# duanyiqun/DiffusionDepth

Measured on AMD Instinct MI355X. Metric: depth-maps/sec (20-step DDIM, KITTI 352x1216 f16r, B=4 maps per GPU per step; depth RMSE vs the reference's CPU path <= 1e-3 on this workload AND at KITTI's depth range 0-80 m: see cpu_baseline.rmse_gate), higher is better.
Workload: dtype f16 (f16 MFMA operands, fp32 accumulation; refined mode: f16-pair weights in conv1 / conv4 / conv3(cond), block-scaled int16 hand-over of y3 and conv3(cond)); 1 GPU; kitti 352x1216 image -> latent 16x176x608, cond 256x176x608, Res head denoiser (mmbev_res50 config), T=20, encoder+loop+decoder, inputs resident in HBM; global_batch=4, parallelism=dp1 (independent images, no collective), ranks_seen=1, streams=2, graph=True, variant=res

## Files before the change

diffusiondepth_amd/csrc/dd_api.cpp:

```cpp
#include "dd_api_internal.h"
#include <cstdlib>

namespace ddapi {
thread_local std::string g_create_error;
}


extern "C" {

const char* dd_version(void) { return "ddepth 0.1 gfx950 (hip, mfma bf16/f16/f32 implicit-GEMM conv3x3+GN+ReLU, hipGraph DDIM loop)"; }

const char* dd_last_error(dd_handle_t h) { return h ? h->err.c_str() : g_create_error.c_str(); }

int dd_create(dd_handle_t* out, int device, int variant) {
  if (!out) { g_create_error = "dd_create: out is NULL"; return DD_ERR_INVALID_ARG; }
  *out = nullptr;
  if (variant != DD_VARIANT_RES && variant != DD_VARIANT_SWIN) { g_create_error = "dd_create: unknown variant"; return DD_ERR_INVALID_ARG; }
  int n = 0;
  hipError_t e = hipGetDeviceCount(&n);
  if (e != hipSuccess || n <= 0) {
    g_create_error = std::string("dd_create: no HIP device available (") + (e != hipSuccess ? hipGetErrorString(e) : "count = 0") +
                     "); this library has no CPU fallback";
    return DD_ERR_HIP;
  }
// ... 82 lines not shown
    h->swin_w5 = (int)value;
  }
  else if (k == "hoist_cond") {
    if (value < -1 || value > 1) return h->fail(DD_ERR_INVALID_ARG, "dd_set_option: hoist_cond must be -1 (automatic), 0 or 1");
    h->hoist_cond = (int)value;
  }
  else if (k == "bf16_storage") {
    if (h->bf16_pure != (value != 0)) {
      DD_HIP(hipDeviceSynchronize());
      h->plans.clear(); h->last_once_plan = nullptr;
      h->cond_bufs.clear(); h->fpn_cond.reset(); h->fpn_cond_key[3] = -1; h->fpn_out.reset(); h->fpn_work.reset();
    }
    h->bf16_pure = value != 0;
  }
  else if (k == "naive_wgrad") h->naive_wgrad = value != 0;
  else if (k == "lane_probe") h->lane_probe = value != 0;
  else if (k == "x3_grad_fp32") h->x3_grad_fp32 = value != 0;
  else if (k == "grad_autoscale") h->grad_autoscale = value != 0;
  else if (k == "keep_trajectory") h->keep_traj = value != 0;
  else if (k == "use_trajectory") h->use_traj = value;
  else if (k == "adjoint_tiled") h->adjoint_tiled = value != 0;
  else if (k == "streams") h->n_streams = value < 1 ? 1 : (int)value;
  else if (k == "keep_activations_mb") h->keep_act_mb = value < 0 ? 0 : value;
  else if (k == "big_tiles") {
    if (value < -1 || value > 1) return h->fail(DD_ERR_INVALID_ARG, "dd_set_option: big_tiles must be -1 (automatic), 0 or 1");
    if (h->big_tiles != (int)value) { DD_HIP(hipDeviceSynchronize()); h->plans.clear(); h->last_once_plan = nullptr; }
    h->big_tiles = (int)value;
  }
  else if (k == "thin_slots") {
    if (value < 1 || value > 4096) return h->fail(DD_ERR_INVALID_ARG, "dd_set_option: thin_slots must be in [1, 4096]");
    if (h->thin_slots != (int)value) { DD_HIP(hipDeviceSynchronize()); h->plans.clear(); h->last_once_plan = nullptr; }
    h->thin_slots = (int)value;
  }
  else if (k == "one_buffer") {
    if (value < 0 || value > 2) return h->fail(DD_ERR_INVALID_ARG, "dd_set_option: one_buffer must be 0, 1 or 2");
    if (h->one_buffer != (int)value) { DD_HIP(hipDeviceSynchronize()); h->plans.clear(); h->last_once_plan = nullptr; }
    h->one_buffer = (int)value;
  }
  else if (k == "cond_direct") {
    if (value < 0 || value > 1) return h->fail(DD_ERR_INVALID_ARG, "dd_set_option: cond_direct must be 0 or 1");
    h->cond_direct = (int)value;
  }
  else if (k == "cond_split") {
    if (value < 0 || value > 1) return h->fail(DD_ERR_INVALID_ARG, "dd_set_option: cond_split must be 0 or 1");
    h->cond_split = (int)value;
  }
  else if (k == "thin_stream") {
    if (value < 0 || value > 1) return h->fail(DD_ERR_INVALID_ARG, "dd_set_option: thin_stream must be 0 or 1");
    if (h->thin_stream != (int)value) {
      DD_HIP(hipDeviceSynchronize());
      h->plans.clear(); h->last_once_plan = nullptr;
    }
    h->thin_stream = (int)value;
  }
  else if (k == "f16r_wide" || k == "f16r_p4" || k == "f16r_c1") {
    if (value < 0 || value > 1) return h->fail(DD_ERR_INVALID_ARG, "dd_set_option: " + k + " must be 0 or 1");
    int& opt = k == "f16r_wide" ? h->f16r_wide : k == "f16r_c1" ? h->f16r_c1 : h->f16r_p4;
    if (opt != (int)value) { DD_HIP(hipDeviceSynchronize()); h->plans.clear(); h->last_once_plan = nullptr; }
    opt = (int)value;
  }
  else if (k == "phase_prof_buffer") h->prof_buf = reinterpret_cast<unsigned long long*>((uintptr_t)value);
  else if (k == "phase_prof_layer") h->prof_layer = (int)value;
  else if (k == "layer_timing") {
    drain_layer_events(h);
    h->layer_timing = value != 0;
    for (int i = 0; i < dd_handle_s::N_LAYER_SLOTS; ++i) { h->layer_ms[i] = 0; h->layer_cnt[i] = 0; }
  } else return h->fail(DD_ERR_INVALID_ARG, "dd_set_option: unknown key '" + k + "'");
  return DD_OK;
}

int dd_get_counter(dd_handle_t h, const char* key, int64_t* value) {
  if (!h || !key || !value) return DD_ERR_INVALID_ARG;
  const std::string k(key);
  if (k == "graph_launches") *value = h->n_graph_launches;
  else if (k == "graph_default") *value = h->graph_off_by_env ? 0 : 1;
  else if (k == "eager_loops") *value = h->n_eager_loops;
  else if (k == "graph_capture_failures") *value = h->n_capture_failures;
  else if (k == "plans") *value = (int64_t)h->plans.size();
  else if (k == "neck_launches") *value = h->n_neck_launches;
  else if (k == "trajectory_ticket") *value = h->traj_serial;
  else if (k == "lane_calls") *value = h->n_lane_calls;
  else if (k == "lane_probe_retries") *value = h->n_lane_probe_retries;
  else if (k == "lane_overlap") *value = h->lane_overlap_seen;
  else if (k == "cond_split_ok") *value = (h->fpn_committed && h->fpn_split_ok ? 1 : 0) | (h->neck_committed && h->neck_split_ok ? 2 : 0);
  else if (k == "resident_slots") *value = h->resident_slots;
  else if (k == "trajectory_reuses") *value = h->n_traj_reuse;
  else if (k == "thin_stream_launches") *value = h->thin_stream_launches;
  else if (k.compare(0, 13, "kid_launches:") == 0) {
    int id = 0;
    const size_t n = k.size() - 13;
    bool ok = n >= 1 && n <= 3 && !(n > 1 && k[13] == '0');
    for (size_t i = 13; ok && i < k.size(); ++i) { ok = k[i] >= '0' && k[i] <= '9'; id = id * 10 + (k[i] - '0'); }
    if (!ok || !kid_listed(id)) return h->fail(DD_ERR_INVALID_ARG, "dd_get_counter: '" + k + "' does not name a kernel id (dd_kernel_ids.h)");
    *value = h->kid_launches[id];
  }
  else return h->fail(DD_ERR_INVALID_ARG, "dd_get_counter: unknown key '" + k + "'");
  return DD_OK;
}

int dd_get_layer_ms(dd_handle_t h, int layer, double* total_ms, int64_t* launches) {
  if (!h || layer < 1 || layer > dd_handle_s::N_LAYER_SLOTS || !total_ms || !launches) return DD_ERR_INVALID_ARG;
  drain_layer_events(h);
  *total_ms = h->layer_ms[layer - 1];
  *launches = h->layer_cnt[layer - 1];
  return DD_OK;
}

int dd_last_loop_ms(dd_handle_t h, float* ms) {
  if (!h || !ms) return DD_ERR_INVALID_ARG;
  *ms = 0.f;
  if (!h->ev_valid) return DD_OK;
  DD_HIP(hipEventSynchronize(h->ev1));
  DD_HIP(hipEventElapsedTime(ms, h->ev0, h->ev1));
  return DD_OK;
}

static int condition_impl(dd_handle_t h, const float* const* feats, const int* feat_h, const int* feat_w, int n_levels, int B,
                          float* cond_out, int precision, void* stream, bool with_neck);

int dd_condition(dd_handle_t h, const float* const* feats, const int* feat_h, const int* feat_w, int n_levels, int B,
                 float* cond_out, int precision, void* stream) {
  return condition_impl(h, feats, feat_h, feat_w, n_levels, B, cond_out, precision, stream, false);
}

int dd_neck_condition(dd_handle_t h, const float* const* feats, const int* feat_h, const int* feat_w, int n_levels, int B,
                      float* cond_out, int precision, void* stream) {
  if (!h) return DD_ERR_INVALID_ARG;
  if (!h->neck_committed) return h->fail(DD_ERR_STATE, "hahineck.* weights not committed (dd_set_weight for the lateral / projection / fusion convolutions, "
                                                       "dd_commit_weights; DD_VARIANT_SWIN)");
  return condition_impl(h, feats, feat_h, feat_w, n_levels, B, cond_out, precision, stream, true);
}

static int condition_impl(dd_handle_t h, const float* const* feats, const int* feat_h, const int* feat_w, int n_levels, int B,
                          float* cond_out, int precision, void* stream, bool with_neck) {
  if (!h) return DD_ERR_INVALID_ARG;
  if (!h->fpn_committed) return h->fail(DD_ERR_STATE, "conv_lateral.* / conv_up.* weights not committed (dd_set_weight, dd_commit_weights)");
  if (with_neck && h->variant != DD_VARIANT_SWIN)
    return h->fail(DD_ERR_UNSUPPORTED, "dd_neck_condition: the HAHI neck kernels are built for the Swin-L (192/384/768/1536) and MPViT-small (128/216/288/288) pyramids of DD_VARIANT_SWIN");
  if (n_levels != FPN_LEVELS || !feats || !feat_h || !feat_w) return h->fail(DD_ERR_INVALID_ARG, "dd_condition: expects 4 pyramid levels");
  if (precision < DD_PREC_FP32 || precision > DD_PREC_LAST) return h->fail(DD_ERR_INVALID_ARG, "dd_condition: precision must be fp32, bf16, f16, f16x3 or f16r");
// ... 522 lines not shown
```

diffusiondepth_amd/csrc/dd_api_internal.h:

```cpp
#pragma once
#include "../../include/ddepth.h"
#include "dd_kernels.h"
#include "dd_kernel_ids.h"

#include <cmath>
#include <cstdio>
#include <cstring>
#include <list>
#include <map>
#include <memory>
#include <set>
#include <string>
#include <tuple>
#include <vector>

using namespace dd;

namespace ddapi {

extern thread_local std::string g_create_error;

struct DevBuf {
  void* p = nullptr;
  size_t bytes = 0;
// ... 41 lines not shown
enum { PYR_DEFAULT = 0, PYR_MPVIT = 1 };
inline int pyramid_of(int variant, int pyr) { return pyr == PYR_MPVIT ? PYRAMID_MPVIT : variant == DD_VARIANT_SWIN ? PYRAMID_SWIN : PYRAMID_RES; }
inline const int* fpn_cin(int variant, int pyr) {
  return pyr == PYR_MPVIT ? FPN_CIN_MPVIT : (variant == DD_VARIANT_SWIN ? FPN_CIN_SWIN : FPN_CIN_RES);
}
inline const int* fpn_cin_pad(int variant, int pyr) { return pyr == PYR_MPVIT ? FPN_CIN_MPVIT_PAD : fpn_cin(variant, pyr); }

struct ConvLayer {
  int cin = 0, cout = 0;
  DevBuf wpack2[NUM_WIMG];
  DevBuf bias;
  DevBuf w_oihw;
  DevBuf wpackT[NUM_EK];
  DevBuf wT_oihw;
  DevBuf gamma, beta;
};

struct PlanKey {
  int B, h, w, ch, cw, T, prec, hoist;
  int keep = 0;
  int lane = 0;
  int lanes = 1;
  bool operator<(const PlanKey& o) const {
    return std::tie(B, h, w, ch, cw, T, prec, hoist, keep, lane, lanes) < std::tie(o.B, o.h, o.w, o.ch, o.cw, o.T, o.prec, o.hoist, o.keep, o.lane, o.lanes);
  }
};

struct Plan {
  PlanKey key{};
  int ek = EK_F32;
  DevBuf x[2];
  std::shared_ptr<DevBuf> cond;
  const void* cond_alias = nullptr;
  const void* graph_cond = nullptr;
  void* cond_ptr() const { return cond_alias ? const_cast<void*>(cond_alias) : (cond ? cond->p : nullptr); }
  DevBuf y1, y2, y3, y4;
  DevBuf a1, f, a3, eps;
  DevBuf sa, sf;
  DevBuf bX, bA1, bF, bA3;
  DevBuf bSa, bSf;
  DevBuf xstash;
  int64_t traj_ticket = 0;
  int64_t traj_weights = -1;
  bool traj_consumed = false;
  DevBuf gA, gY;
  DevBuf dgb;
  DevBuf bcorr;
  DevBuf ttab, tt_scratch;
  int64_t ttab_weights = -1;
  DevBuf ccond;
  DevBuf ccond_raw;
  DevBuf ccond_scale;
  DevBuf y3_scale;
  bool wide = false, c1 = false, p4 = false;
  DevBuf stats;
  DevBuf c1c2;
  DevBuf tsteps;
  std::vector<long long> tsteps_host;
  size_t stats_bytes = 0;
  hipGraphExec_t exec = nullptr;
  bool capture_failed = false;
  uint64_t last_use = 0;
  ~Plan() { if (exec) (void)hipGraphExecDestroy(exec); }
  int slots = 1;
  size_t kept_bytes = 0;
  void* slot(const DevBuf& b, int step) const { return static_cast<char*>(b.p) + (slots > 1 ? (size_t)step * (b.bytes / slots) : 0); }
  double* stat_ptr(int step, int layer) const {
    return stats.as<double>() + ((size_t)(step * 4 + layer) * key.B) * STAT_SLOTS * STAT_STRIDE;
  }
};

struct FpnWork {
  int B = 0, ek = -1, pyr = 0, hs[FPN_LEVELS] = {0}, ws[FPN_LEVELS] = {0};
  DevBuf fin[FPN_LEVELS];
  DevBuf lat[FPN_LEVELS];
  DevBuf up[FPN_LEVELS - 1];
  DevBuf pooled[FPN_LEVELS - 1];
  bool neck = false;
  DevBuf nk_cat[FPN_LEVELS];
  DevBuf nk_out[FPN_LEVELS];
};


struct NeckConv { int layer; std::string name; int cout, cin, ks, level, kind, C, Ck; };
constexpr int NECK_C_MPVIT[4] = {128, 216, 288, 288};
inline int neck_c(int pyr, int level) { return pyr == PYR_MPVIT ? NECK_C_MPVIT[level] : (192 << level); }
inline int neck_ck(int pyr, int level) { return pyr == PYR_MPVIT ? FPN_CIN_MPVIT_PAD[level] : (192 << level); }
inline std::vector<NeckConv> neck_convs(int pyr) {
  std::vector<NeckConv> v;
  const int P = pyramid_of(DD_VARIANT_SWIN, pyr);
  for (int i = 0; i < 4; ++i) {
    const int C = neck_c(pyr, i), Ck = neck_ck(pyr, i);
    const std::string si = std::to_string(i), sj = std::to_string(i - 1);
    v.push_back({kid_neck(P, NECK_LATERAL, i), "hahineck.lateral_convs." + si, C, C, 1, i, NECK_LATERAL, C, Ck});
    v.push_back({kid_neck(P, NECK_PROJ, i), i == 0 ? std::string("hahineck.conv_proj.0") : "hahineck.trans_proj." + sj, 512, C, 1, i, NECK_PROJ, C, Ck});
    v.push_back({kid_neck(P, NECK_FUSION, i), i == 0 ? std::string("hahineck.conv_fusion.0") : "hahineck.trans_fusion." + sj, C, C + 512, 3, i, NECK_FUSION, C, Ck});
  }
  return v;
}

}
using namespace ddapi;


struct dd_handle_s {
  static constexpr int MAX_LANES = 4;
  int device = 0;
  int variant = DD_VARIANT_RES;
  std::string err;
  std::map<std::string, std::vector<float>> host_w;
  std::map<std::string, std::unique_ptr<DevBuf>> dev_w;
  std::set<std::string> dev_newer;
  DevBuf stage;
  bool committed = false;
  bool codec_committed = false;
  ConvLayer L[4];
  ConvLayer LA, LB;
  DevBuf emb;
  DevBuf etab;
  DevBuf w5_oihw, w5pack[NUM_WIMG], pairp, kside;
  int64_t w5_weights = -1;
  int swin_w5 = 1;
  DevBuf zero_bias;
  int hoist_cond = -1;
  bool bf16_pure = false;
  DevBuf codec_buf;
  CodecWeights codec{};
  DevBuf codec_tmp;
  std::vector<float> acp;
  DevBuf d_acp;
  int n_train = 0;
  bool use_graph = true, timing = false, debug_sync = false, layer_timing = false;
  bool graph_off_by_env = false;
  int graph_fence = 0;
  bool train_graphs = false;
  int check_finite = 0;
  DevBuf chk_buf; std::vector<std::string> chk_labels;
  int ablate = 0;
  unsigned long long* prof_buf = nullptr;
  int prof_layer = 0;
  bool keep_traj = false;
  int64_t keep_act_mb = 65536;
  int n_streams = 1;
  int thin_slots = 512;
  int big_tiles = -1;
  int one_buffer = 1;
  int thin_stream = 1;
  int f16r_wide = 1;
  int f16r_c1 = 1;
  int f16r_p4 = 0;
  bool split_ok = true;
  DevBuf wmax;
  int resident_slots = 512;
  hipStream_t lane_stream[MAX_LANES] = {nullptr, nullptr, nullptr, nullptr};
  std::vector<hipEvent_t> probe_events;
  std::vector<hipStream_t> burnt_streams;
  int lane_probe = 1;
  int64_t n_lane_probe_retries = 0, lane_overlap_seen = -1;
  hipEvent_t lane_fork = nullptr, lane_done[MAX_LANES] = {nullptr, nullptr, nullptr, nullptr};
  int64_t n_lane_calls = 0;
  int active_lanes = 1;
  bool adjoint_tiled = true;
  int64_t traj_serial = 0, use_traj = 0, weights_serial = 0, n_traj_reuse = 0;
  int naive_wgrad = 0;
  int grad_autoscale = 1;
  DevBuf grad_scale;
  int x3_grad_fp32 = 0;
  std::map<PlanKey, std::unique_ptr<Plan>> plans;
  DevBuf wgrad_ws[MAX_LANES];
  static constexpr int SCALED_SET = MAX_LANES, GRAD_SETS = MAX_LANES + 1;
  std::map<std::string, std::unique_ptr<DevBuf>> grads[GRAD_SETS];
  std::map<std::tuple<int, int, int, int, int>, std::pair<std::shared_ptr<DevBuf>, uint64_t>> cond_bufs;
  bool neck_committed = false;
  DevBuf neck_w[NECK_CONVS][NUM_WIMG], neck_b[NECK_CONVS];
  int64_t n_neck_launches = 0;
  bool fpn_committed = false;
  int fpn_pyramid = PYR_DEFAULT;
  DevBuf fpn_lat_w[FPN_LEVELS][NUM_WIMG], fpn_lat_b[FPN_LEVELS];
  DevBuf fpn_up_w[FPN_LEVELS - 1][NUM_WIMG], fpn_up_b[FPN_LEVELS - 1];
  std::unique_ptr<FpnWork> fpn_work;
  std::shared_ptr<DevBuf> fpn_out;
  bool fpn_split_ok = false, neck_split_ok = false;
  int cond_direct = 1;
  int cond_split = 1;
  std::shared_ptr<DevBuf> fpn_cond;
  int fpn_cond_key[4] = {0, 0, 0, -1};
  uint64_t tick = 0;
  Plan* last_once_plan = nullptr;
  hipEvent_t ev0 = nullptr, ev1 = nullptr;
  bool ev_valid = false;
  hipStream_t cap_stream = nullptr;
  int64_t n_graph_launches = 0, n_eager_loops = 0, n_capture_failures = 0;
  static constexpr int N_LAYER_SLOTS = KID_LAST;
  double layer_ms[N_LAYER_SLOTS] = {0};
  int64_t layer_cnt[N_LAYER_SLOTS] = {0};
  std::vector<std::tuple<int, hipEvent_t, hipEvent_t>> pending_ev;
  int64_t kid_launches[KID_LAST + 1] = {0};
  int64_t thin_stream_launches = 0;

  int fail(int code, const std::string& m) { err = m; return code; }
};

#define DD_HIP(expr)                                                                              \
  do {                                                                                            \
    hipError_t _e = (expr);                                                                       \
    if (_e != hipSuccess)                                                                         \
      return h->fail(DD_ERR_HIP, std::string(#expr) + ": " + hipGetErrorString(_e));              \
  } while (0)

#define DD_TRY(expr) do { int _rc = (expr); if (_rc != DD_OK) return _rc; } while (0)

namespace ddapi {
struct WeightSpec { std::string name; int64_t numel; };

inline const char* const kConvNames[4] = {"model.noise_embedding.0", "model.noise_embedding.3", "model.pred.0", "model.pred.3"};
inline const char* const kGnNames[4] = {"model.noise_embedding.1", "model.noise_embedding.4", "model.pred.1", "model.pred.4"};
constexpr int kCins[4] = {LATENT_C, HID_C, COND_C, HID_C}, kCouts[4] = {HID_C, COND_C, HID_C, LATENT_C};

int weight_group(const std::string& name);
std::vector<WeightSpec> required_weights(int variant, int pyr = PYR_DEFAULT);
int pack_geom(dd_handle_t h, int kid, int ek, PackGeom* g);
int device_buf(dd_handle_t h, DevBuf& dst, size_t bytes, const void* src = nullptr, hipStream_t s = nullptr);
int pack_images(dd_handle_t h, const float* w, int64_t numel, int kid, const int* slots, int n_slots, DevBuf* images, bool transposed, hipStream_t s);
int check_common(dd_handle_t h, int B, int lh, int lw, int ch, int cw, bool need_schedule);
bool denoiser_image_addressable(int lh, int lw, int ch, int cw);
int lane_count(dd_handle_t h, int B, int precision);
int check_split(dd_handle_t h, int precision, const char* who);
int acquire_lane_stream(dd_handle_t h, int lane, hipStream_t caller);
int get_cond_buf(dd_handle_t h, int B, int lh, int lw, int precision, std::shared_ptr<DevBuf>* out, int lane = 0);
int want_hoist(dd_handle_t h, int precision, int T = 1, int keep = 0);
bool keep2_fits(dd_handle_t h, size_t need);
bool plan_big_tiles(dd_handle_t h, const PlanKey& key);
int get_plan(dd_handle_t h, const PlanKey& key, Plan** out);
bool conv_tiles(ConvParams& p, int kid, int ek);
int launch_conv(dd_handle_t h, int kid, int ek, ConvParams p, hipStream_t s, int slot = 0);
template <class F> hipError_t timed(dd_handle_t h, int slot, hipStream_t s, F launch) {
  if (!h->layer_timing || slot <= 0) return launch();
  hipEvent_t a, b;
  hipError_t e = hipEventCreate(&a); if (e != hipSuccess) return e;
  e = hipEventCreate(&b); if (e != hipSuccess) return e;
  (void)hipEventRecord(a, s);
  e = launch();
  (void)hipEventRecord(b, s);
  h->pending_ev.emplace_back(slot - 1, a, b);
  return e;
}
int enqueue_fused_step(dd_handle_t h, Plan* pl, int step, const float* x_in, float* x_out, bool apply_update,
                       const long long* tvec, int t_base, int t_bstride, hipStream_t s);
int enqueue_naive_eps(dd_handle_t h, Plan* pl, int step, const float* x_in, const long long* tvec, int t_base,
                      int t_bstride, hipStream_t s);
int enqueue_cond_conv(dd_handle_t h, Plan* pl, hipStream_t s, const float* nchw = nullptr);
// ... 18 lines not shown
```

diffusiondepth_amd/csrc/dd_api_plans.cpp:

```cpp
#include "dd_api_internal.h"

#include <algorithm>

namespace ddapi {

int check_common(dd_handle_t h, int B, int lh, int lw, int ch, int cw, bool need_schedule) {
  if (!h) return DD_ERR_INVALID_ARG;
  if (!h->committed) return h->fail(DD_ERR_STATE, "model.* weights not committed (call dd_set_weight for every key, then dd_commit_weights)");
  if (need_schedule && h->n_train <= 0) return h->fail(DD_ERR_STATE, "schedule not set (dd_set_schedule)");
  if (B <= 0 || lh <= 0 || lw <= 0) return h->fail(DD_ERR_INVALID_ARG, "B, lat_h, lat_w must be positive");
  if (h->variant == DD_VARIANT_RES && (ch != lh || cw != lw))
    return h->fail(DD_ERR_INVALID_ARG, "DD_VARIANT_RES needs cond_h,cond_w == lat_h,lat_w (reference ...res.py:340 adds them elementwise)");
  if (h->variant == DD_VARIANT_SWIN && (ch <= 0 || cw <= 0)) return h->fail(DD_ERR_INVALID_ARG, "cond_h, cond_w must be positive");
  if ((long long)B * lh * lw * COND_C >= (1LL << 31) * 4) return h->fail(DD_ERR_INVALID_ARG, "tensor too large");
  if (!denoiser_image_addressable(lh, lw, ch, cw))
    return h->fail(DD_ERR_UNSUPPORTED, "one image's 256-channel fp32 map of " + std::to_string(std::max((long long)lh * lw, (long long)ch * cw)) +
                   " pixels does not fit the 32-bit byte offsets of the convolution kernels' buffer addressing (at most 2^32 - 16 bytes per image and tensor)");
  return DD_OK;
}

bool denoiser_image_addressable(int lh, int lw, int ch, int cw) {
  const unsigned long long px = (unsigned long long)std::max((long long)lh * lw, (long long)ch * cw);
  return px <= (1ull << 40) && conv_buffer_addressable(px * COND_C * 4ull);
}
// ... 95 lines not shown
  return true;
}
int launch_conv(dd_handle_t h, int kid, int ek, ConvParams p, hipStream_t s, int slot) {
  if (!conv_tiles(p, kid, ek)) return h->fail(DD_ERR_INVALID_ARG, "no fused convolution kernel for kernel id " + std::to_string(kid) + " in element kind " + std::to_string(ek));
  DD_HIP(timed(h, slot, s, [&] { return launch_conv_igemm2(kid, ek, p, s); }));
  h->kid_launches[kid_route(kid, ek).id]++;
  return DD_OK;
}

int get_plan(dd_handle_t h, const PlanKey& key, Plan** out) {
  auto it = h->plans.find(key);
  if (it != h->plans.end()) { it->second->last_use = ++h->tick; *out = it->second.get(); return DD_OK; }
  const size_t cap = 10 + 2 * (size_t)(h->n_streams > 1 ? (h->n_streams < dd_handle_s::MAX_LANES ? h->n_streams : dd_handle_s::MAX_LANES) : 0);
  while (h->plans.size() >= cap) {
    auto victim = h->plans.end();
    for (auto j = h->plans.begin(); j != h->plans.end(); ++j) {
      const Plan& q = *j->second;
      if (q.key.keep && q.traj_ticket != 0 && q.traj_weights == h->weights_serial && !q.traj_consumed) continue;
      if (victim == h->plans.end() || q.last_use < victim->second->last_use) victim = j;
    }
    if (victim == h->plans.end()) break;
    if (h->last_once_plan == victim->second.get()) h->last_once_plan = nullptr;
    DD_HIP(hipDeviceSynchronize());
    h->plans.erase(victim);
  }
  std::unique_ptr<Plan> pl(new Plan());
  pl->key = key;
  const bool naive = key.prec == DD_PREC_NAIVE_FP32;
  pl->ek = naive ? EK_F32 : ek_of_precision(key.prec, h->bf16_pure);
  if (pl->ek == EK_F16R && !key.hoist)
    return h->fail(DD_ERR_UNSUPPORTED, "DD_PREC_F16R runs the hoisted forward-only plans: for the Swin / MPViT denoiser those exist with option swin_w5 = 1 "
                                       "(dd_denoise / dd_denoise_trace / dd_denoise_once); training plans: DD_PREC_F16");
  const size_t px = (size_t)key.B * key.h * key.w;
  const size_t es = ek_size(pl->ek);
  DD_HIP(pl->x[0].alloc(px * LATENT_C * 4));
  DD_HIP(pl->x[1].alloc(px * LATENT_C * 4));
  if (key.keep) DD_HIP(pl->xstash.alloc((size_t)(key.T > 0 ? key.T : 1) * px * LATENT_C * 4));
  const bool swin = h->variant == DD_VARIANT_SWIN;
  if (!(pl->ek == EK_F16R && !swin && key.hoist)) { int rc = get_cond_buf(h, key.B, key.h, key.w, key.prec, &pl->cond, key.lane); if (rc) return rc; }
  pl->slots = (key.keep == 2 && key.T > 0) ? key.T : 1;
  const size_t ns = (size_t)pl->slots;
  if (swin) {
    const size_t es_s = pl->ek == EK_F16R ? 4 : es;
    DD_HIP(pl->sa.alloc(ns * px * COND_C * es_s)); DD_HIP(pl->sf.alloc(ns * px * COND_C * es_s));
  }
  if (key.hoist)
  {
    PackGeom g3;
    DD_TRY(pack_geom(h, conv3h_kid(h, key), pl->ek, &g3));
    const int th = g3.th;
    DD_HIP(pl->ccond.alloc((size_t)key.B * ((key.h + th - 1) / th) * ((key.w + 31) / 32) * th * 32 * HID_C * 4));
    if (pl->ek == EK_F16R) {
      pl->wide = h->f16r_wide != 0; pl->c1 = h->f16r_c1 != 0; pl->p4 = h->f16r_p4 != 0;
      DD_HIP(pl->ccond_raw.alloc((size_t)key.B * ((key.h + 7) / 8) * ((key.w + 31) / 32) * 8 * 32 * HID_C * 4));
      if (pl->wide) DD_HIP(pl->ccond_scale.alloc((size_t)key.B * ((key.h + th - 1) / th) * ((key.w + 31) / 32) * 4 * 2 * (th / 4) * 4));
    }
  }
  if (key.hoist && swin) {
    const int T1 = key.T > 0 ? key.T : key.B;
    const int RH = key.h < SWIN_TT_AX ? key.h : SWIN_TT_AX, RW = key.w < SWIN_TT_AX ? key.w : SWIN_TT_AX;
    DD_HIP(pl->ttab.alloc((size_t)T1 * SWIN_TT_ROWS * HID_C * 4));
    DD_HIP(pl->tt_scratch.alloc((size_t)T1 * RH * RW * (2 * COND_C + HID_C) * 4));
    if (h->swin_w5) {
      DD_HIP(pl->bcorr.alloc((size_t)key.B * swin_ring_stride(key.h, key.w) * HID_C * 4));
      DD_HIP(hipMemsetAsync(pl->bcorr.p, 0, pl->bcorr.bytes, nullptr));
      DD_HIP(hipStreamSynchronize(nullptr));
    }
  }
  DD_HIP(pl->y1.alloc(ns * px * HID_C * es));
  DD_HIP(pl->y2.alloc(ns * px * COND_C * es));
  DD_HIP(pl->y3.alloc(ns * px * HID_C * es));
  if (pl->ek == EK_F16R && h->f16r_wide) DD_HIP(pl->y3_scale.alloc(ns * px * 4));
  DD_HIP(pl->y4.alloc(ns * px * LATENT_C * 4));
  if (key.keep == 2) pl->kept_bytes = pl->y1.bytes + pl->y2.bytes + pl->y3.bytes + pl->y3_scale.bytes + pl->y4.bytes + pl->sa.bytes + pl->sf.bytes;
  if (naive) {
    DD_HIP(pl->a1.alloc(px * HID_C * 4));
    DD_HIP(pl->f.alloc(px * COND_C * 4));
    DD_HIP(pl->a3.alloc(px * HID_C * 4));
    DD_HIP(pl->eps.alloc(px * LATENT_C * 4));
  }
  const int T = key.T > 0 ? key.T : 1;
  pl->stats_bytes = (size_t)(T + 1) * 4 * key.B * STAT_SLOTS * STAT_STRIDE * sizeof(double);
  DD_HIP(pl->stats.alloc(pl->stats_bytes));
  std::vector<float> c1c2((size_t)T * 2, 0.f);
  std::vector<long long> ts((size_t)T, 0);
  if (key.T > 0) {
    const int ratio = h->n_train / key.T;
    for (int k = 0; k < key.T; ++k) {
      const int t = (key.T - 1 - k) * ratio;
      const int prev = t - ratio;
      const double a_t = (double)h->acp[t];
      const double a_prev = prev >= 0 ? (double)h->acp[prev] : 1.0;
      c1c2[2 * k] = (float)std::sqrt(a_prev / a_t);
      c1c2[2 * k + 1] = (float)(std::sqrt(1.0 - a_prev) - std::sqrt(a_prev * (1.0 - a_t) / a_t));
      ts[k] = t;
    }
  }
  DD_HIP(pl->c1c2.alloc(c1c2.size() * 4));
  DD_HIP(pl->tsteps.alloc(ts.size() * 8));
  pl->tsteps_host = ts;
  DD_HIP(hipMemcpy(pl->c1c2.p, c1c2.data(), c1c2.size() * 4, hipMemcpyHostToDevice));
  DD_HIP(hipMemcpy(pl->tsteps.p, ts.data(), ts.size() * 8, hipMemcpyHostToDevice));
  pl->last_use = ++h->tick;
  *out = pl.get();
  h->plans[key] = std::move(pl);
  return DD_OK;
}
// ... 71 lines not shown
    DD_TRY(timed_launch(KID_SWIN_CONVB, p));
    p.in = sf_; p.wpack = h->L[2].wpack2[wk].p; p.bias = h->L[2].bias.as<float>(); p.out = y3_;
    p.stats_out = pl->stat_ptr(step, 2);
    DD_TRY(timed_launch(KID_SWIN_PRED, p));
  } else {
  p.in = y2_; p.wpack = h->L[2].wpack2[wk].p; p.bias = h->L[2].bias.as<float>(); p.out = y3_;
  p.stats_out = pl->stat_ptr(step, 2); p.stats_in = pl->stat_ptr(step, 1);
  p.gn_gamma = h->L[1].gamma.as<float>(); p.gn_beta = h->L[1].beta.as<float>();
  p.cond = pl->cond_ptr(); p.emb = h->emb.as<float>(); p.tvec = tvec; p.t_base = t_base; p.t_bstride = t_bstride;
  p.cadd = pl->ccond.as<float>(); p.etab = h->etab.as<float>();
  p.cadd_scale = pl->ccond_scale.as<float>(); p.out_scale = static_cast<float*>(pl->slot(pl->y3_scale, step));
  DD_TRY(timed_launch(k.hoist ? KID_CONV3H : KID_CONV3, p));
  p.cadd_scale = nullptr; p.out_scale = nullptr;
  }
  p.in = y3_; p.wpack = h->L[3].wpack2[rf ? WIMG_STACK : wimg_slot(tk)].p; p.bias = h->L[3].bias.as<float>(); p.out = y4_;
  p.stats_out = pl->stat_ptr(step, 3); p.stats_in = pl->stat_ptr(step, 2);
  p.gn_gamma = h->L[2].gamma.as<float>(); p.gn_beta = h->L[2].beta.as<float>();
  DD_TRY(timed_launch(KID_CONV4, p));
  if (h->debug_sync) DD_HIP(hipStreamSynchronize(s));
  return DD_OK;
}

int enqueue_naive_eps(dd_handle_t h, Plan* pl, int step, const float* x_in, const long long* tvec, int t_base,
                      int t_bstride, hipStream_t s) {
  const PlanKey& k = pl->key;
  const int B = k.B, hh = k.h, ww = k.w;
  auto L = h->L;
  DD_HIP(launch_naive_conv3x3(x_in, L[0].w_oihw.as<float>(), L[0].bias.as<float>(), pl->y1.as<float>(), B, hh, ww, LATENT_C, HID_C, s));
  DD_HIP(launch_naive_gn_stats(pl->y1.as<float>(), pl->stat_ptr(step, 0), B, hh, ww, HID_C, s));
  DD_HIP(launch_naive_gn_apply(pl->y1.as<float>(), pl->stat_ptr(step, 0), L[0].gamma.as<float>(), L[0].beta.as<float>(),
                               nullptr, nullptr, nullptr, 0, 0, pl->a1.as<float>(), B, hh, ww, HID_C, s));
  DD_HIP(launch_naive_conv3x3(pl->a1.as<float>(), L[1].w_oihw.as<float>(), L[1].bias.as<float>(), pl->y2.as<float>(), B, hh, ww, HID_C, COND_C, s));
  DD_HIP(launch_naive_gn_stats(pl->y2.as<float>(), pl->stat_ptr(step, 1), B, hh, ww, COND_C, s));
  DD_HIP(launch_naive_gn_apply(pl->y2.as<float>(), pl->stat_ptr(step, 1), L[1].gamma.as<float>(), L[1].beta.as<float>(),
                               static_cast<const float*>(pl->cond_ptr()), h->emb.as<float>(), tvec, t_base, t_bstride, pl->f.as<float>(), B, hh, ww, COND_C, s));
  DD_HIP(launch_naive_conv3x3(pl->f.as<float>(), L[2].w_oihw.as<float>(), L[2].bias.as<float>(), pl->y3.as<float>(), B, hh, ww, COND_C, HID_C, s));
  DD_HIP(launch_naive_gn_stats(pl->y3.as<float>(), pl->stat_ptr(step, 2), B, hh, ww, HID_C, s));
  DD_HIP(launch_naive_gn_apply(pl->y3.as<float>(), pl->stat_ptr(step, 2), L[2].gamma.as<float>(), L[2].beta.as<float>(),
                               nullptr, nullptr, nullptr, 0, 0, pl->a3.as<float>(), B, hh, ww, HID_C, s));
  DD_HIP(launch_naive_conv3x3(pl->a3.as<float>(), L[3].w_oihw.as<float>(), L[3].bias.as<float>(), pl->y4.as<float>(), B, hh, ww, HID_C, LATENT_C, s));
  DD_HIP(launch_naive_gn_stats(pl->y4.as<float>(), pl->stat_ptr(step, 3), B, hh, ww, LATENT_C, s));
  DD_HIP(launch_naive_gn_apply(pl->y4.as<float>(), pl->stat_ptr(step, 3), L[3].gamma.as<float>(), L[3].beta.as<float>(),
                               nullptr, nullptr, nullptr, 0, 0, pl->eps.as<float>(), B, hh, ww, LATENT_C, s));
  if (h->debug_sync) DD_HIP(hipStreamSynchronize(s));
  return DD_OK;
}

int enqueue_cond_conv(dd_handle_t h, Plan* pl, hipStream_t s, const float* nchw) {
  const PlanKey& k = pl->key;
  ConvParams p{};
  p.B = k.B; p.h = k.h; p.w = k.w;
  if (pl->ek == EK_F16R) {
    p.in = nchw ? static_cast<const void*>(nchw) : pl->cond_ptr(); p.wpack = h->L[2].wpack2[WIMG_SPLIT].p; p.bias = h->zero_bias.as<float>();
    p.out = pl->ccond_raw.p;
    DD_TRY(launch_conv(h, nchw ? CONV3C_NCHW : KID_CONV3C, EK_F16S, p, s));
    DD_HIP(launch_cadd_reformat(pl->ccond_raw.as<float>(), pl->ccond.p, pl->ccond_scale.as<float>(), k.B, k.h, k.w, plan_big_tiles(h, k) ? 1 : 0, pl->wide ? 2 : 1, s));
    return DD_OK;
  }
  p.in = pl->cond_ptr(); p.wpack = h->L[2].wpack2[wimg_slot(thin_kind(pl->ek))].p; p.bias = h->zero_bias.as<float>(); p.out = pl->ccond.p;
  return launch_conv(h, conv3c_kid(h, k), pl->ek, p, s);
}


int ensure_swin_w5(dd_handle_t h, hipStream_t s) {
  if (h->w5_weights == h->weights_serial) return DD_OK;
  if (!h->LB.w_oihw.p || !h->L[2].w_oihw.p) return h->fail(DD_ERR_STATE, "hoisted Swin form: the fp32 weights of convB / pred.0 are not on the device");
  if (!h->w5_oihw.p) {
    DD_HIP(h->w5_oihw.alloc((size_t)HID_C * COND_C * 25 * 4)); DD_HIP(h->pairp.alloc((size_t)81 * COND_C * HID_C * 4)); DD_HIP(h->kside.alloc(SWIN_KSIDE_BYTES));
  }
  DD_HIP(launch_swin_compose(h->LB.w_oihw.as<float>(), h->L[2].w_oihw.as<float>(), h->w5_oihw.as<float>(), h->pairp.as<float>(), h->kside.p, s));
  DD_TRY(pack_images(h, h->w5_oihw.as<float>(), (int64_t)HID_C * COND_C * 25, SWIN_PRED5_H, kImageSlots, 4, h->w5pack, false, s));
  h->w5_weights = h->weights_serial;
  return DD_OK;
}

int enqueue_swin_hoist(dd_handle_t h, Plan* pl, hipStream_t s) {
  const PlanKey& k = pl->key;
  if (k.T > 0 && pl->ttab_weights != h->weights_serial) {
    if (!h->LA.w_oihw.p || !h->LB.w_oihw.p || !h->L[2].w_oihw.p) return h->fail(DD_ERR_STATE, "hoisted Swin form: the fp32 weights of the fuse convolutions are not on the device");
    DD_HIP(launch_swin_ttab(h->LA.w_oihw.as<float>(), h->LB.w_oihw.as<float>(), h->L[2].w_oihw.as<float>(), h->emb.as<float>(),
                            pl->tsteps.as<long long>(), k.T, k.h, k.w, pl->tt_scratch.as<float>(), pl->ttab.as<float>(), s));
    pl->ttab_weights = h->weights_serial;
  }
  if (pl->bcorr.p) { int rc = ensure_swin_w5(h, s); if (rc) return rc; }
  ConvParams p{};
  p.B = k.B; p.h = k.h; p.w = k.w;
  if (pl->ek == EK_F16R) {
    p.in = pl->cond_ptr(); p.wpack = h->LA.wpack2[WIMG_SPLIT].p; p.bias = h->LA.bias.as<float>(); p.out = pl->sa.p;
    DD_TRY(launch_conv(h, KID_SWIN_CONVB, EK_F16S, p, s));
    p.in = pl->sa.p; p.wpack = h->LB.wpack2[WIMG_SPLIT].p; p.bias = h->LB.bias.as<float>(); p.out = pl->sf.p;
    DD_TRY(launch_conv(h, KID_SWIN_CONVB, EK_F16S, p, s));
    p.in = pl->sf.p; p.wpack = h->L[2].wpack2[WIMG_SPLIT].p; p.bias = h->zero_bias.as<float>(); p.out = pl->ccond_raw.p;
    DD_TRY(launch_conv(h, KID_CONV3C, EK_F16S, p, s));
    DD_HIP(launch_cadd_reformat(pl->ccond_raw.as<float>(), pl->ccond.p, pl->ccond_scale.as<float>(), k.B, k.h, k.w, plan_big_tiles(h, k) ? 1 : 0, pl->wide ? 2 : 1, s));
    return DD_OK;
  }
  const int tk = thin_kind(pl->ek);
  p.in = pl->cond_ptr(); p.wpack = h->LA.wpack2[wimg_slot(tk)].p; p.bias = h->LA.bias.as<float>(); p.out = pl->sa.p;
  DD_TRY(launch_conv(h, KID_SWIN_CONVB, tk, p, s));
  p.in = pl->sa.p; p.wpack = h->LB.wpack2[wimg_slot(tk)].p; p.bias = h->LB.bias.as<float>(); p.out = pl->sf.p;
  DD_TRY(launch_conv(h, KID_SWIN_CONVB, tk, p, s));
  p.in = pl->sf.p; p.wpack = h->L[2].wpack2[wimg_slot(tk)].p; p.bias = h->zero_bias.as<float>(); p.out = pl->ccond.p;
  return launch_conv(h, conv3c_kid(h, k), pl->ek, p, s);
}

int stage_condition(dd_handle_t h, Plan* pl, const float* cond, int B, int lat_h, int lat_w, int cond_h, int cond_w,
// ... 66 lines not shown
```

diffusiondepth_amd/csrc/dd_igemm2.hip:

```cpp
#include "dd_igemm2_cfg.h"
#include "dd_gcn.h"

namespace dd {

#if DD_PHASE_PROF && !defined(DD_HOST_EMULATION)
#define DD_PROF_MARK(i) do { if (p.prof != nullptr && threadIdx.x == 0) p.prof[(size_t)blockIdx.x * 8 + (i)] = (unsigned long long)wall_clock64(); } while (0)
#define DD_PROF_HWID() do { if (p.prof != nullptr && threadIdx.x == 0) {                                                     \
    unsigned hw_, xcc_; asm volatile("s_getreg_b32 %0, hwreg(HW_REG_HW_ID)" : "=s"(hw_)); asm volatile("s_getreg_b32 %0, hwreg(HW_REG_XCC_ID)" : "=s"(xcc_));   \
    p.prof[(size_t)blockIdx.x * 8 + 6] = hw_; p.prof[(size_t)blockIdx.x * 8 + 7] = xcc_; } } while (0)
#define DD_PROF_CLK() ((unsigned long long)__builtin_amdgcn_s_memtime())
#define DD_PROF_LOOP_DECL unsigned long long pl_acc_[4] = {0, 0, 0, 0}, pl_t_ = 0
#define DD_PROF_LOOP_START() do { if (p.prof != nullptr) pl_t_ = DD_PROF_CLK(); } while (0)
#define DD_PROF_LOOP_ADD(k) do { if (p.prof != nullptr) { const unsigned long long n_ = DD_PROF_CLK(); pl_acc_[k] += n_ - pl_t_; pl_t_ = n_; } } while (0)
#define DD_PROF_LOOP_STORE() do { if (p.prof != nullptr && lane == 0) { for (int k_ = 0; k_ < 4; ++k_)                          \
    p.prof[(size_t)gridDim.x * 8 + ((size_t)blockIdx.x * C::WAVES + wave) * 4 + k_] = pl_acc_[k_]; } } while (0)
#else
#define DD_PROF_MARK(i) ((void)0)
#define DD_PROF_HWID() ((void)0)
#define DD_PROF_LOOP_DECL
#define DD_PROF_LOOP_START() ((void)0)
#define DD_PROF_LOOP_ADD(k) ((void)0)
#define DD_PROF_LOOP_STORE() ((void)0)
#endif

// ... 17 lines not shown
  const int li = lane & 31, g = lane >> 5;
  DD_PROF_MARK(0);
  DD_PROF_HWID();

  constexpr int NSPLIT = C::COUT_PAD / C::NT;
  int wgid;
  {
    const int nwg = gridDim.x, bid = blockIdx.x;
    const int xcd = bid & 7, q = nwg >> 3, r = nwg & 7;
    wgid = (xcd < r ? xcd * (q + 1) : r * (q + 1) + (xcd - r) * q) + (bid >> 3);
  }
  constexpr int NSPLIT_G = NSPLIT / C::SPW;
  const int nsplit = (wgid % NSPLIT_G) * C::SPW;
  const int tiles_per_img = p.tiles_x * p.tiles_y;
#ifndef DD_SPLIT_FLIP
#define DD_SPLIT_FLIP 1
#endif
  const int flip = (DD_SPLIT_FLIP && C::SPW == 2) ? ((wgid / NSPLIT_G) & 1) : 0;
  int n0 = (nsplit + flip) * C::NT;
  int sbase = 0;
  const int h = p.h, w = p.w;
  const bool have_norm = (C::PRO == PRO_X) ? (p.step > 0) : (C::PRO != PRO_RAW);
  const int abl = DD_ABLATE ? p.ablate : 0;
  if (abl & 256) return;
  int tile = wgid / NSPLIT_G;
  int b, y0, x0;
  const char *in_b, *cond_b, *y4_b;
  char* xout_b;
  dd_buf_t in_d, cond_d, y4_d, xout_d;
  auto set_tile_base = [&](int t) {
    tile = t;
    b = t / tiles_per_img;
    const int trem = t - b * tiles_per_img;
    const int ty = trem / p.tiles_x, tx = trem - ty * p.tiles_x;
    y0 = ty * C::TH; x0 = tx * C::TW;
    if constexpr (C::IS_NECK) {
      const int cs = p.in_cstride ? p.in_cstride : C::CIN;
      in_b = reinterpret_cast<const char*>(p.in) + ((size_t)b * cs + p.in_coff) * h * w * IN_ESZ;
    } else {
      in_b = reinterpret_cast<const char*>(p.in) + (size_t)b * h * w * C::CIN * IN_ESZ;
    }
    cond_b = (C::PRO == PRO_GN_ADD) ? reinterpret_cast<const char*>(p.cond) + (size_t)b * h * w * C::CIN * IN_ESZ : nullptr;
    y4_b = (C::PRO == PRO_X) ? reinterpret_cast<const char*>(p.y4) + (size_t)b * h * w * LATENT_C * 4 : nullptr;
    xout_b = (C::PRO == PRO_X) ? reinterpret_cast<char*>(p.xout) + (size_t)b * h * w * LATENT_C * 4 : nullptr;
    in_d = dd_make_buf(in_b, (unsigned long long)h * w * C::CIN * IN_ESZ);
    cond_d = dd_make_buf(cond_b, (C::PRO == PRO_GN_ADD) ? (unsigned long long)h * w * C::CIN * IN_ESZ : 0ull);
    y4_d = dd_make_buf(y4_b, (C::PRO == PRO_X) ? (unsigned long long)h * w * LATENT_C * 4 : 0ull);
    xout_d = dd_make_buf(xout_b, (C::PRO == PRO_X) ? (unsigned long long)h * w * LATENT_C * 4 : 0ull);
  };
  set_tile_base(tile);

  const unsigned lds_base = DD_LDS_BASE(smem);
  constexpr int W_KIB = C::W_BYTES / 1024;
  constexpr int NWPIECE = (W_KIB + C::WAVES - 1) / C::WAVES;
  constexpr bool W_EVEN = W_KIB % C::WAVES == 0 && NWPIECE <= 4;
  const dd_bufw_t w_d = dd_make_bufw(reinterpret_cast<const char*>(p.wpack) + (size_t)nsplit * C::NSTAGE * (size_t)C::W_BYTES, (unsigned long long)C::SPW * C::NSTAGE * C::W_BYTES);
  const unsigned lane16 = lane * 16;
  auto issue_weights = [&](int s) {
    const int si = flip ? (s < C::NSTAGE ? s + C::NSTAGE : s - C::NSTAGE) : s;
    const unsigned src = (unsigned)si * C::W_BYTES;
    const unsigned dst = lds_base + C::W_OFF + (s & (C::NWB - 1)) * C::W_BYTES;
    if constexpr (W_EVEN) {
      const unsigned first = wave * (NWPIECE * 1024);
      dd_buf_lds_dma16<NWPIECE>(smem, w_d, lane16, __builtin_amdgcn_readfirstlane(src + first), __builtin_amdgcn_readfirstlane(dst + first));
    } else {
#pragma unroll
      for (int c = 0; c < NWPIECE; ++c) {
        const int kc = c * C::WAVES + wave;
        if (kc < W_KIB) dd_buf_lds_dma16<1>(smem, w_d, lane16, __builtin_amdgcn_readfirstlane(src + kc * 1024), __builtin_amdgcn_readfirstlane(dst + kc * 1024));
      }
    }
  };

  const int jfix = tid & (PPP - 1);
  int lds_off[NIT];
  unsigned voff[NIT];
  unsigned m_valid = 0, m_inside = 0, m_interior = 0;
  auto set_tile_geometry = [&]() {
    m_valid = 0; m_inside = 0; m_interior = 0;
#pragma unroll
    for (int u = 0; u < NIT; ++u) {
      const int it = u * C::THREADS + tid;
      const int itc = it < C::ITEMS ? it : C::ITEMS - 1;
      const int pp = itc >> C::LOG2_PPP;
      const int pr = pp / PW, pc = pp - pr * PW;
      const int gy = y0 - C::HALO + pr, gx = x0 - C::HALO + pc;
      const bool inside = gy >= 0 && gy < h && gx >= 0 && gx < w;
      if (it < C::ITEMS) m_valid |= 1u << u;
      if (inside) m_inside |= 1u << u;
      if (inside && pr >= C::HALO && pr < C::HALO + C::TH && pc >= C::HALO && pc < C::HALO + C::TW) m_interior |= 1u << u;
      const int gyc = gy < 0 ? 0 : (gy >= h ? h - 1 : gy);
      const int gxc = gx < 0 ? 0 : (gx >= w ? w - 1 : gx);
      const unsigned pix = (unsigned)(gyc * w + gxc), lc = (unsigned)(jfix * EPP);
      if constexpr (C::IN_NCHW) voff[u] = (lc * h * w + pix) * 4u;
      else if constexpr (C::CIN >= ACT_CB) voff[u] = (((lc >> 5) * h * w + pix) * ACT_CB + (lc & (ACT_CB - 1))) * IN_ESZ;
      else voff[u] = (pix * C::CIN + lc) * IN_ESZ;
      lds_off[u] = pp * ROWB + ((jfix << 4) ^ swz16<RPB, PPP>(pc));
    }
  };
  set_tile_geometry();

  constexpr int RD = C::RAW_DEPTH;
  uint4 raw[RD][NIT][NLD];
  uint4 aux[NIT][NLD];
  auto load_raw = [&](int chunk, int slot) {
    static_assert(CK == 16 || CK % ACT_CB == 0, "channel chunk against the 32-channel blocks");
    const unsigned cb = (unsigned)chunk * CK;
    if constexpr (C::IN_NCHW) {
      static_assert(EPP == 8 && NLD == 2 && C::PRO == PRO_RAW, "fp32 source, eight channels per piece, no auxiliary tensor");
      const unsigned HW4 = (unsigned)h * w * 4u;
#pragma unroll
      for (int u = 0; u < NIT; ++u) {
#pragma unroll
        for (int q = 0; q < NLD; ++q)
          raw[slot][u][q] = make_uint4(dd_buf_load4(in_d, voff[u], (cb + 4 * q + 0) * HW4, 0), dd_buf_load4(in_d, voff[u], (cb + 4 * q + 1) * HW4, 0),
                                       dd_buf_load4(in_d, voff[u], (cb + 4 * q + 2) * HW4, 0), dd_buf_load4(in_d, voff[u], (cb + 4 * q + 3) * HW4, 0));
      }
      DD_VMEM_LOADS_ISSUED(NIT * NLD * 4);
      return;
    }
    const unsigned soff = (C::CIN >= ACT_CB) ? ((cb >> 5) * h * w * ACT_CB + (cb & (ACT_CB - 1))) * IN_ESZ : cb * IN_ESZ;
#pragma unroll
// ... 487 lines not shown
                a4[0] = t4.x; a4[1] = t4.y; a4[2] = t4.z; a4[3] = t4.w;
              } else {
                const uint2 t2 = *reinterpret_cast<const uint2*>(ab);
                if constexpr (EK == EK_BF16) {
                  a4[0] = bf16_to_f32(t2.x & 0xFFFFu); a4[1] = bf16_to_f32(t2.x >> 16); a4[2] = bf16_to_f32(t2.y & 0xFFFFu); a4[3] = bf16_to_f32(t2.y >> 16);
                } else {
                  a4[0] = f16_to_f32(t2.x & 0xFFFFu); a4[1] = f16_to_f32(t2.x >> 16); a4[2] = f16_to_f32(t2.y & 0xFFFFu); a4[3] = f16_to_f32(t2.y >> 16);
                }
              }
#pragma unroll
              for (int i = 0; i < 4; ++i) v[i] += a4[i];
            }
          }
        }
    };
    if constexpr (C::Q15) {
      float pmax = 0.f;
#pragma unroll
      for (int n = 0; n < C::WN; ++n)
#pragma unroll
        for (int q = 0; q < 4; ++q) {
          float v[4];
          value_of(n, q, v);
          if (pvalid) {
            const float s = (v[0] + v[1]) + (v[2] + v[3]);
            const float sq = fmaf(v[0], v[0], fmaf(v[1], v[1], fmaf(v[2], v[2], v[3] * v[3])));
            const int lg = 2 * n + (q >> 1);
            ls[lg] += s; lq[lg] += sq;
          }
          pmax = fmaxf(pmax, fmaxf(fmaxf(fabsf(v[0]), fabsf(v[1])), fmaxf(fabsf(v[2]), fabsf(v[3]))));
#pragma unroll
          for (int i = 0; i < 4; ++i) acc[n][m][q * 4 + i] = v[i];
        }
      pmax = fmaxf(pmax, __shfl_xor(pmax, 32, 64));
      const float inv = pmax > 0.f ? 1.f / pmax : 0.f;
      if (pvalid && g == 0) p.out_scale[(size_t)e_b * h * w + (size_t)gy * w + gx] = pmax * (1.f / Q15_ONE);
#pragma unroll
      for (int n = 0; n < C::WN; ++n) {
        uint2 pk[4];
#pragma unroll
        for (int q = 0; q < 4; ++q) {
          pk[q].x = DD_CVT_PKNORM_I16(acc[n][m][q * 4 + 0] * inv, acc[n][m][q * 4 + 1] * inv);
          pk[q].y = DD_CVT_PKNORM_I16(acc[n][m][q * 4 + 2] * inv, acc[n][m][q * 4 + 3] * inv);
        }
#pragma unroll
        for (int k = 0; k < 2; ++k) {
          const auto rx = __builtin_amdgcn_permlane32_swap(pk[2 * k].x, pk[2 * k + 1].x, false, false);
          const auto ry = __builtin_amdgcn_permlane32_swap(pk[2 * k].y, pk[2 * k + 1].y, false, false);
          if (pvalid) dd_buf_store16(out_d, out_v, ((n0 >> 5) + n) * out_blk + m * out_row, 32 * k, make_uint4(rx[0], ry[0], rx[1], ry[1]));
        }
      }
      continue;
    }
#pragma unroll
    for (int n = 0; n < C::WN; ++n) {
      uint2 pk[4];
#pragma unroll
      for (int q = 0; q < 4; ++q) {
        if (C::COUT < 32 && q >= 2) continue;
        const int co = n0 + n * 32 + 8 * q + 4 * g;
        float v[4];
        value_of(n, q, v);
        if (C::STATS && pvalid) {
          const float s = (v[0] + v[1]) + (v[2] + v[3]);
          const float sq = fmaf(v[0], v[0], fmaf(v[1], v[1], fmaf(v[2], v[2], v[3] * v[3])));
          const int lg = (C::COUT == COND_C) ? (n >> 1) : (C::COUT == HID_C) ? (2 * n + (q >> 1)) : q;
          ls[lg] += s; lq[lg] += sq;
        }
        if constexpr (C::LAYER == KID_CONV3C) {
          const size_t fi = ((((size_t)e_tile * C::WAVES + wave) * C::WN + n) * C::WM + m) * 256 + q * 64 + lane;
          if constexpr (C::CADD16) reinterpret_cast<uint2*>(p.out)[fi] = make_uint2(pack2<EK_F16>(v[0], v[1]), pack2<EK_F16>(v[2], v[3]));
          else reinterpret_cast<float4*>(p.out)[fi] = make_float4(v[0], v[1], v[2], v[3]);
        } else if constexpr (C::OUT_ESZ == 4) {
          if (pvalid && (C::COUT_PAD == C::COUT || co < C::COUT)) {
            if constexpr (C::SCATTER) {
              const int par = co >> 8, cc = co & (COND_C - 1);
              *reinterpret_cast<float4*>(reinterpret_cast<char*>(p.out) + ((size_t)e_b * 4 * h * w * COND_C +
                  act_offset(COND_C, 2 * h, 2 * w, 0, cc, 2 * gy + (par >> 1), 2 * gx + (par & 1))) * 4) = make_float4(v[0], v[1], v[2], v[3]);
            } else {
              dd_buf_store16(out_d, out_v, ((n0 >> 5) + n) * out_blk + m * out_row, 32 * q, make_uint4(__builtin_bit_cast(uint32_t, v[0]), __builtin_bit_cast(uint32_t, v[1]),
                                                                                                       __builtin_bit_cast(uint32_t, v[2]), __builtin_bit_cast(uint32_t, v[3])));
            }
          }
        } else {
          pk[q].x = pack2<C::OUT_K>(v[0], v[1]);
          pk[q].y = pack2<C::OUT_K>(v[2], v[3]);
        }
      }
      if constexpr (C::OUT_ESZ == 2) {
#pragma unroll
        for (int k = 0; k < 2; ++k) {
          const auto rx = __builtin_amdgcn_permlane32_swap(pk[2 * k].x, pk[2 * k + 1].x, false, false);
          const auto ry = __builtin_amdgcn_permlane32_swap(pk[2 * k].y, pk[2 * k + 1].y, false, false);
          const int co = n0 + n * 32 + 16 * k + 8 * g;
          if (pvalid && (C::COUT_PAD == C::COUT || co < C::COUT)) {
            if constexpr (C::SCATTER) {
              const int par = co >> 8, cc = co & (COND_C - 1);
              *reinterpret_cast<uint4*>(reinterpret_cast<char*>(p.out) + ((size_t)e_b * 4 * h * w * COND_C +
                  act_offset(COND_C, 2 * h, 2 * w, 0, cc, 2 * gy + (par >> 1), 2 * gx + (par & 1))) * 2) = make_uint4(rx[0], ry[0], rx[1], ry[1]);
            } else {
              dd_buf_store16(out_d, out_v, ((n0 >> 5) + n) * out_blk + m * out_row, 32 * k, make_uint4(rx[0], ry[0], rx[1], ry[1]));
            }
          }
        }
      }
    }
// ... 103 lines not shown
```

Baseline: 550.9 maps/s.

## Fuse block-scaled int16 quantization of conv3(cond) into the conv epilogue

On the wide f16r path, the cond conv3 epilogue now computes a per-block absmax across the wave, writes the scale, and stores int16-normalized values straight into the ccond buffer. This drops the fp32 ccond_raw intermediate and the separate cadd_reformat launch. The weight-DMA issue is also generalized: each wave copies a contiguous run in chunks of four, and the remainder is spread across waves, replacing the old even/uneven split. The risk is that block order and scale semantics must match the old reformat kernel exactly, and the wave-wide shuffle reduction adds some epilogue cost.

```diff
diff --git a/diffusiondepth_amd/csrc/dd_api.cpp b/diffusiondepth_amd/csrc/dd_api.cpp
--- a/diffusiondepth_amd/csrc/dd_api.cpp
+++ b/diffusiondepth_amd/csrc/dd_api.cpp
@@ -158,6 +158,14 @@
       h->plans.clear(); h->last_once_plan = nullptr;
     }
     h->thin_stream = (int)value;
+  }
+  else if (k == "cond_quant_epilogue") {
+    if (value < 0 || value > 1) return h->fail(DD_ERR_INVALID_ARG, "dd_set_option: cond_quant_epilogue must be 0 or 1");
+    if (h->cond_quant_epilogue != (int)value) {
+      DD_HIP(hipDeviceSynchronize());
+      h->plans.clear(); h->last_once_plan = nullptr;
+    }
+    h->cond_quant_epilogue = (int)value;
   }
   else if (k == "f16r_wide" || k == "f16r_p4" || k == "f16r_c1") {
     if (value < 0 || value > 1) return h->fail(DD_ERR_INVALID_ARG, "dd_set_option: " + k + " must be 0 or 1");
@@ -192,6 +200,7 @@
   else if (k == "resident_slots") *value = h->resident_slots;
   else if (k == "trajectory_reuses") *value = h->n_traj_reuse;
   else if (k == "thin_stream_launches") *value = h->thin_stream_launches;
+  else if (k == "cond_quant_launches") *value = h->cond_quant_launches;
   else if (k.compare(0, 13, "kid_launches:") == 0) {
     int id = 0;
     const size_t n = k.size() - 13;
diff --git a/diffusiondepth_amd/csrc/dd_api_internal.h b/diffusiondepth_amd/csrc/dd_api_internal.h
--- a/diffusiondepth_amd/csrc/dd_api_internal.h
+++ b/diffusiondepth_amd/csrc/dd_api_internal.h
@@ -117,6 +117,7 @@
   DevBuf ccond_raw;
   DevBuf ccond_scale;
   DevBuf y3_scale;
+  bool cq = false;
   bool wide = false, c1 = false, p4 = false;
   DevBuf stats;
   DevBuf c1c2;
@@ -210,6 +211,7 @@
   int thin_slots = 512;
   int big_tiles = -1;
   int one_buffer = 1;
+  int cond_quant_epilogue = 1;
   int thin_stream = 1;
   int f16r_wide = 1;
   int f16r_c1 = 1;
@@ -262,6 +264,7 @@
   std::vector<std::tuple<int, hipEvent_t, hipEvent_t>> pending_ev;
   int64_t kid_launches[KID_LAST + 1] = {0};
   int64_t thin_stream_launches = 0;
+  int64_t cond_quant_launches = 0;
 
   int fail(int code, const std::string& m) { err = m; return code; }
 };
diff --git a/diffusiondepth_amd/csrc/dd_api_plans.cpp b/diffusiondepth_amd/csrc/dd_api_plans.cpp
--- a/diffusiondepth_amd/csrc/dd_api_plans.cpp
+++ b/diffusiondepth_amd/csrc/dd_api_plans.cpp
@@ -171,7 +171,8 @@
     DD_HIP(pl->ccond.alloc((size_t)key.B * ((key.h + th - 1) / th) * ((key.w + 31) / 32) * th * 32 * HID_C * 4));
     if (pl->ek == EK_F16R) {
       pl->wide = h->f16r_wide != 0; pl->c1 = h->f16r_c1 != 0; pl->p4 = h->f16r_p4 != 0;
-      DD_HIP(pl->ccond_raw.alloc((size_t)key.B * ((key.h + 7) / 8) * ((key.w + 31) / 32) * 8 * 32 * HID_C * 4));
+      pl->cq = h->cond_quant_epilogue != 0 && pl->wide && !swin && th == 8;
+      if (!pl->cq) DD_HIP(pl->ccond_raw.alloc((size_t)key.B * ((key.h + 7) / 8) * ((key.w + 31) / 32) * 8 * 32 * HID_C * 4));
       if (pl->wide) DD_HIP(pl->ccond_scale.alloc((size_t)key.B * ((key.h + th - 1) / th) * ((key.w + 31) / 32) * 4 * 2 * (th / 4) * 4));
     }
   }
@@ -349,6 +350,12 @@
   p.B = k.B; p.h = k.h; p.w = k.w;
   if (pl->ek == EK_F16R) {
     p.in = nchw ? static_cast<const void*>(nchw) : pl->cond_ptr(); p.wpack = h->L[2].wpack2[WIMG_SPLIT].p; p.bias = h->zero_bias.as<float>();
+    if (pl->cq) {
+      p.out = pl->ccond.p; p.out_scale = pl->ccond_scale.as<float>();
+      DD_TRY(launch_conv(h, nchw ? CONV3C_NCHW : KID_CONV3C, EK_F16S, p, s));
+      h->cond_quant_launches++;
+      return DD_OK;
+    }
     p.out = pl->ccond_raw.p;
     DD_TRY(launch_conv(h, nchw ? CONV3C_NCHW : KID_CONV3C, EK_F16S, p, s));
     DD_HIP(launch_cadd_reformat(pl->ccond_raw.as<float>(), pl->ccond.p, pl->ccond_scale.as<float>(), k.B, k.h, k.w, plan_big_tiles(h, k) ? 1 : 0, pl->wide ? 2 : 1, s));
diff --git a/diffusiondepth_amd/csrc/dd_igemm2.hip b/diffusiondepth_amd/csrc/dd_igemm2.hip
--- a/diffusiondepth_amd/csrc/dd_igemm2.hip
+++ b/diffusiondepth_amd/csrc/dd_igemm2.hip
@@ -93,22 +93,27 @@
 
   const unsigned lds_base = DD_LDS_BASE(smem);
   constexpr int W_KIB = C::W_BYTES / 1024;
-  constexpr int NWPIECE = (W_KIB + C::WAVES - 1) / C::WAVES;
-  constexpr bool W_EVEN = W_KIB % C::WAVES == 0 && NWPIECE <= 4;
+  constexpr int W_RUN = W_KIB / C::WAVES, W_REM = W_KIB % C::WAVES;
   const dd_bufw_t w_d = dd_make_bufw(reinterpret_cast<const char*>(p.wpack) + (size_t)nsplit * C::NSTAGE * (size_t)C::W_BYTES, (unsigned long long)C::SPW * C::NSTAGE * C::W_BYTES);
   const unsigned lane16 = lane * 16;
   auto issue_weights = [&](int s) {
     const int si = flip ? (s < C::NSTAGE ? s + C::NSTAGE : s - C::NSTAGE) : s;
     const unsigned src = (unsigned)si * C::W_BYTES;
     const unsigned dst = lds_base + C::W_OFF + (s & (C::NWB - 1)) * C::W_BYTES;
-    if constexpr (W_EVEN) {
-      const unsigned first = wave * (NWPIECE * 1024);
-      dd_buf_lds_dma16<NWPIECE>(smem, w_d, lane16, __builtin_amdgcn_readfirstlane(src + first), __builtin_amdgcn_readfirstlane(dst + first));
-    } else {
-#pragma unroll
-      for (int c = 0; c < NWPIECE; ++c) {
-        const int kc = c * C::WAVES + wave;
-        if (kc < W_KIB) dd_buf_lds_dma16<1>(smem, w_d, lane16, __builtin_amdgcn_readfirstlane(src + kc * 1024), __builtin_amdgcn_readfirstlane(dst + kc * 1024));
+    if constexpr (W_RUN > 0) {
+      const unsigned first = wave * (W_RUN * 1024);
+      const unsigned src0 = __builtin_amdgcn_readfirstlane(src + first), dst0 = __builtin_amdgcn_readfirstlane(dst + first);
+#pragma unroll
+      for (int c = 0; c < W_RUN; c += 4) {
+        constexpr int LEFT = W_RUN % 4;
+        if (c + 4 <= W_RUN) dd_buf_lds_dma16<4>(smem, w_d, lane16, src0 + c * 1024, dst0 + c * 1024);
+        else dd_buf_lds_dma16<LEFT ? LEFT : 4>(smem, w_d, lane16, src0 + c * 1024, dst0 + c * 1024);
+      }
+    }
+    if constexpr (W_REM > 0) {
+      if (wave < W_REM) {
+        const unsigned rest = (C::WAVES * W_RUN + wave) * 1024;
+        dd_buf_lds_dma16<1>(smem, w_d, lane16, __builtin_amdgcn_readfirstlane(src + rest), __builtin_amdgcn_readfirstlane(dst + rest));
       }
     }
   };
@@ -702,6 +707,36 @@
       }
       continue;
     }
+    if constexpr (C::LAYER == KID_CONV3C && C::SPLIT) {
+      static_assert(C::WAVES == 4 && C::WN == 2 && C::WM == 2 && !C::CADD16, "the block order of the loop's 8x32-tile conv3 (ConvParams::cadd_scale)");
+      if (p.out_scale != nullptr) {
+        auto nmax = [](float a, float b) { return (b > a || b != b) ? b : a; };
+#pragma unroll
+        for (int n = 0; n < C::WN; ++n) {
+          float4 v4[4];
+#pragma unroll
+          for (int q = 0; q < 4; ++q) {
+            float v[4];
+            value_of(n, q, v);
+            v4[q] = make_float4(v[0], v[1], v[2], v[3]);
+          }
+          float mx = nmax(nmax(fabsf(v4[0].x), fabsf(v4[0].y)), nmax(fabsf(v4[0].z), fabsf(v4[0].w)));
+#pragma unroll
+          for (int q = 1; q < 4; ++q) mx = nmax(mx, nmax(nmax(fabsf(v4[q].x), fabsf(v4[q].y)), nmax(fabsf(v4[q].z), fabsf(v4[q].w))));
+#pragma unroll
+          for (int off = 32; off >= 1; off >>= 1) mx = nmax(mx, __shfl_xor(mx, off, 64));
+          const float inv = mx > 0.f ? 1.f / mx : 0.f;
+          const size_t blk = (((size_t)e_tile * C::WAVES + wave) * C::WN + n) * C::WM + m;
+          if (lane == 0) p.out_scale[blk] = mx * (1.f / Q15_ONE);
+#pragma unroll
+          for (int q = 0; q < 4; ++q) {
+            const float4 v = v4[q];
+            reinterpret_cast<uint2*>(p.out)[blk * 256 + q * 64 + lane] = make_uint2(DD_CVT_PKNORM_I16(v.x * inv, v.y * inv), DD_CVT_PKNORM_I16(v.z * inv, v.w * inv));
+          }
+        }
+        continue;
+      }
+    }
 #pragma unroll
     for (int n = 0; n < C::WN; ++n) {
       uint2 pk[4];
```

Result: no change. 553.5 maps/s, median of 6 (+0.5%).
